# hir0shim/singleSpMV

Hardware: AMD Instinct MI355X
Metric: SpMV GFLOP/s (fp64) + achieved HBM GB/s (higher is better)
Workload: dtype f64

## Files before the change

### singlespmv_amd/csrc/k_bin.hip

```cpp
#include "device.hpp"
#include "internal.hpp"

namespace spmv {

typedef uint32_t bin_u32x4 __attribute__((ext_vector_type(4)));

template <int U>
struct MulBatch {
    double v[U];
    uint32_t c[U];
    int32_t d[U];
};

template <int U, int PL, int MODE, bool LONG>
__device__ __forceinline__ void mul_load(MulBatch<U> &B, int64_t base, int64_t e0, int64_t e1, int lane,
                                         const double *__restrict__ val1, const uint16_t *__restrict__ cs1,
                                         const int32_t *__restrict__ dst1, int64_t ls, int64_t lsh,
                                         const int32_t *__restrict__ lcode) {
    if constexpr (!LONG) {
        const double *vb = val1 + base + lane;
        const uint16_t *cb = cs1 + base + lane;
        const int32_t *db = dst1 + ((base + lane) >> PL);
#pragma unroll
        for (int u = 0; u < U; ++u) {
            B.v[u] = ld_stream(vb + u * 64);
            B.c[u] = (uint32_t)__builtin_nontemporal_load(cb + u * 64);
            if constexpr ((MODE & 4) == 0) B.d[u] = ld_stream(db + u * (64 >> PL));
        }
        (void)e0;
        (void)e1;
        (void)ls;
        (void)lsh;
        (void)lcode;
        (void)db;
    } else {
#pragma unroll
        for (int u = 0; u < U; ++u) {
            const int64_t e = base + u * 64 + lane;
            const int64_t ee = e < e1 ? e : e0;
            B.v[u] = ld_stream(val1 + ee);
            B.c[u] = (uint32_t)__builtin_nontemporal_load(cs1 + ee);
            if (base + u * 64 >= ls) B.d[u] = ld_stream(lcode + (e < e1 ? e + lsh : 0));
            else if constexpr ((MODE & 4) == 0) B.d[u] = ld_stream(dst1 + (ee >> PL));
        }
    }
}

__device__ __forceinline__ void mul_long_block(double pr, int32_t code, bool ok, int lane,
                                               double *__restrict__ prod) {
    const bool start = code < 0 || !ok;
    const uint64_t starts = __ballot(start);
    const uint64_t upto = starts & (~0ull >> (63 - lane));
    const int seg = 63 - __clzll((long long)upto);
    const int r16 = lane & 15, row = lane >> 4;
    double v = ok ? pr : 0.0, t;
    t = dpp_f64<0x111, 0xF>(v);
    if (r16 >= 1 && lane - 1 >= seg) v = __dadd_rn(t, v);
    t = dpp_f64<0x112, 0xF>(v);
    if (r16 >= 2 && lane - 2 >= seg) v = __dadd_rn(t, v);
    t = dpp_f64<0x114, 0xF>(v);
    if (r16 >= 4 && lane - 4 >= seg) v = __dadd_rn(t, v);
    t = dpp_f64<0x118, 0xF>(v);
    if (r16 >= 8 && lane - 8 >= seg) v = __dadd_rn(t, v);
    t = dpp_f64<0x142, 0xA>(v);
    if ((row & 1) && seg <= row * 16 - 1) v = __dadd_rn(t, v);
    t = dpp_f64<0x143, 0xC>(v);
    if (row >= 2 && seg <= 31) v = __dadd_rn(t, v);
    const int32_t pos = code & 0x7FFFFFFF;
    if (ok && pos != 0x7FFFFFFF) prod[pos] = v;
}

template <int U, int MODE, int PL, bool LONG>
__device__ __forceinline__ void mul_store(const MulBatch<U> &B, int64_t base, int64_t e1, int lane,
                                          const double *xs, double *__restrict__ prod, int64_t ls) {
#pragma unroll
    for (int u = 0; u < U; ++u) {
        const int64_t e = base + u * 64 + lane;
        if (LONG && base + u * 64 >= ls) {
            mul_long_block(__dmul_rn(B.v[u], xs[B.c[u]]), B.d[u], e < e1, lane, prod);
        } else if (e < e1) {
            const double pr = __dmul_rn(B.v[u], xs[B.c[u]]);
            double *dp = (MODE & 4) ? prod + e : prod + ((int64_t)B.d[u] << PL) + (e & ((1 << PL) - 1));
            if (MODE & 1) __builtin_nontemporal_store(pr, dp);
            else *dp = pr;
        }
    }
}

template <int U, int MODE, int PL, bool LONG>
__global__ __launch_bounds__(kBinMulThreads) void bin_mul_kernel(
    const int64_t *__restrict__ piece_off, int64_t q_base, const int32_t *__restrict__ piece_strip,
    const int64_t *__restrict__ piece_begin, const int64_t *__restrict__ piece_end,
    const double *__restrict__ val1, const uint16_t *__restrict__ cs1, const int32_t *__restrict__ dst1,
    const double *__restrict__ x, int64_t n, int32_t strip, double *__restrict__ prod,
    const int64_t *__restrict__ lstart, const int64_t *__restrict__ lshift, const int32_t *__restrict__ lcode,
    int32_t xburst) {
    __shared__ double xs[kBinMaxStrip];
    constexpr int NW = kBinMulThreads / 64;
    constexpr int64_t STEP = (int64_t)NW * 64 * U;
    const int w = __builtin_amdgcn_readfirstlane(threadIdx.x >> 6);
    const int lane = threadIdx.x & 63;
    const int64_t q0 = piece_off[q_base + blockIdx.x], q1 = piece_off[q_base + blockIdx.x + 1];
    for (int64_t q = q0; q < q1; ++q) {
        const int32_t st = piece_strip[q];
        const int64_t c0 = (int64_t)st * strip;
        const int64_t e0 = piece_begin[q], e1 = piece_end[q];
        const int64_t ls = LONG ? lstart[st] : INT64_MAX, lsh = LONG ? lshift[st] : 0;
        const int cw = (int)(n - c0 < strip ? n - c0 : strip);
        __syncthreads();
        constexpr int XL = 8;
        if constexpr ((MODE & 256) != 0) {
            const int full = cw & ~127;
            for (int k = w; k * 128 < full; k += NW)
                __builtin_amdgcn_global_load_lds(
                    (const __attribute__((address_space(1))) void *)(x + c0 + k * 128 + lane * 2),
                    (__attribute__((address_space(3))) void *)(xs + k * 128), 16, 0, 0);
            for (int i = full + threadIdx.x; i < cw; i += kBinMulThreads) xs[i] = x[c0 + i];
            __builtin_amdgcn_s_waitcnt(0x0F70);
        } else if (LONG || !xburst) {
            for (int i = threadIdx.x; i < cw; i += kBinMulThreads) xs[i] = x[c0 + i];
        } else for (int i0 = threadIdx.x; i0 < cw; i0 += XL * kBinMulThreads) {
            double t[XL];
#pragma unroll
            for (int k = 0; k < XL; ++k) {
                const int i = i0 + k * kBinMulThreads;
                t[k] = i < cw ? x[c0 + i] : 0.0;
            }
#pragma unroll
            for (int k = 0; k < XL; ++k) {
                const int i = i0 + k * kBinMulThreads;
                if (i < cw) xs[i] = t[k];
            }
        }
        __syncthreads();
        const int64_t first = e0 + (int64_t)w * 64 * U;
        const int64_t nit = first < e1 ? (e1 - first + STEP - 1) / STEP : 0;
        auto bat = [&](int64_t j) { return first + j * STEP; };
        MulBatch<U> A, B;
        if (nit > 0) mul_load<U, PL, MODE, LONG>(A, bat(0), e0, e1, lane, val1, cs1, dst1, ls, lsh, lcode);
        for (int64_t it = 0; it < nit; it += 2) {
            const int64_t ba = bat(it), bb = bat(it + 1);
            if (it + 1 < nit) mul_load<U, PL, MODE, LONG>(B, bb, e0, e1, lane, val1, cs1, dst1, ls, lsh, lcode);
            mul_store<U, MODE, PL, LONG>(A, ba, e1, lane, xs, prod, ls);
            if (it + 1 < nit) {
                if (it + 2 < nit)
                    mul_load<U, PL, MODE, LONG>(A, bat(it + 2), e0, e1, lane, val1, cs1, dst1, ls, lsh, lcode);
                mul_store<U, MODE, PL, LONG>(B, bb, e1, lane, xs, prod, ls);
            }
        }
    }
}

template <int U>
struct SumBatch {
    double v[U];
    uint32_t w[U / 2];
    __device__ __forceinline__ uint32_t slot(int u) const { return (w[u >> 1] >> (16 * (u & 1))) & 0xFFFFu; }
};

template <int U>
__device__ __forceinline__ void sum_load(SumBatch<U> &B, int64_t base, int lane, int64_t pbase, int64_t sbase,
                                         const uint16_t *__restrict__ slot2, const double *__restrict__ prod) {
    static_assert(U % 8 == 0, "slots are read 8 per 16-byte load");
    const bin_u32x4 *sp = reinterpret_cast<const bin_u32x4 *>(slot2 + sbase + (int64_t)lane * 8);
#pragma unroll
    for (int q = 0; q < U / 8; ++q) {
        const bin_u32x4 w = __builtin_nontemporal_load(sp + q * 64);
#pragma unroll
        for (int h = 0; h < 4; ++h) B.w[4 * q + h] = w[h];
    }
    const double *pp = prod + (base - pbase) + lane;
#pragma unroll
    for (int u = 0; u < U; ++u) B.v[u] = ld_stream(pp + u * 64);
}

template <int U>
__device__ __forceinline__ void sum_add(const SumBatch<U> &B, double *ys) {
#pragma unroll
    for (int u = 0; u < U; ++u) atomicAdd(&ys[B.slot(u)], B.v[u]);
}

template <int W2, int U>
__global__ __launch_bounds__(64 * W2) void bin_sum_kernel(
    int64_t b0, int64_t b1, int64_t nbins, int64_t nblk, const int64_t *__restrict__ run_off,
    const int64_t *__restrict__ srun_off, const int32_t *__restrict__ bin_row0, int64_t pbase,
    const uint16_t *__restrict__ slot2,
    const double *__restrict__ prod, double *__restrict__ y) {
    constexpr int SLICE = kBinLdsDoubles / W2;
    constexpr int64_t STEP = 64 * U;
    __shared__ double ylds[kBinLdsDoubles];
    const int w = __builtin_amdgcn_readfirstlane(threadIdx.x >> 6);
    const int lane = threadIdx.x & 63;
    double *ys = ylds + w * SLICE;
    const int64_t bfirst = b0 + (int64_t)blockIdx.x * W2 + w, bstride = (int64_t)gridDim.x * W2;
    if (bfirst >= b1) return;
    int64_t cb = bfirst, k = 0, pos = run_off[cb], end = run_off[cb + 1], rs = pos, ss = srun_off[cb];
    auto next = [&](int64_t &lo, int64_t &sb, int64_t &bb) -> bool {
        while (pos >= end) {
            if (++k >= nblk) {
                cb += bstride;
                if (cb >= b1) return false;
                k = 0;
                pos = rs = run_off[cb];
                end = run_off[cb + 1];
                ss = srun_off[cb];
                continue;
            }
            pos = rs = run_off[k * nbins + cb];
            end = run_off[k * nbins + cb + 1];
            ss = srun_off[k * nbins + cb];
        }
        lo = pos;
        sb = ss + (lo - rs);
        bb = cb;
        pos = pos + STEP < end ? pos + STEP : end;
        return true;
    };
    int64_t acc = -1, done = bfirst;
    auto write_zero = [&](int64_t bz) {
        const int64_t r0 = bin_row0[bz];
        const int rows = (int)(bin_row0[bz + 1] - r0);
        for (int i = lane; i < rows; i += 64) __builtin_nontemporal_store(0.0, y + r0 + i);
    };
    auto finish = [&]() {
        const int64_t r0 = bin_row0[acc];
        const int rows = (int)(bin_row0[acc + 1] - r0);
        __builtin_amdgcn_fence(__ATOMIC_SEQ_CST, "wavefront");
        for (int i = lane; i < rows; i += 64) __builtin_nontemporal_store(ys[i], y + r0 + i);
        __builtin_amdgcn_fence(__ATOMIC_SEQ_CST, "wavefront");
        done = acc + bstride;
    };
    auto begin = [&](int64_t nb) {
        if (nb == acc) return;
        if (acc >= 0) finish();
        for (; done < nb; done += bstride) write_zero(done);
        const int rows = (int)(bin_row0[nb + 1] - bin_row0[nb]);
        for (int i = lane; i < rows; i += 64) ys[i] = 0.0;
        acc = nb;
        done = nb + bstride;
    };
    SumBatch<U> A, B;
    int64_t alo, asb, ab, blo, bsb, bbn;
    bool has_a = next(alo, asb, ab);
    if (has_a) sum_load<U>(A, alo, lane, pbase, asb, slot2, prod);
    while (has_a) {
        const bool has_b = next(blo, bsb, bbn);
        if (has_b) sum_load<U>(B, blo, lane, pbase, bsb, slot2, prod);
        begin(ab);
        sum_add<U>(A, ys);
        if (!has_b) break;
        has_a = next(alo, asb, ab);
        if (has_a) sum_load<U>(A, alo, lane, pbase, asb, slot2, prod);
        begin(bbn);
        sum_add<U>(B, ys);
    }
    if (acc >= 0) finish();
    for (; done < b1; done += bstride) write_zero(done);
}

template <int U>
struct SumTab {
    int32_t t[U / 8];
};

template <int U>
__device__ __forceinline__ void sum_mo_tab(SumTab<U> &T, int64_t sb, int lane, const int32_t *__restrict__ mtab) {
    static_assert(U == 32, "U/8 = 4 table words per lane: one 16-byte load");
    const bin_u32x4 w = __builtin_nontemporal_load(reinterpret_cast<const bin_u32x4 *>(mtab + (sb >> 3)) + lane);
#pragma unroll
    for (int h = 0; h < 4; ++h) T.t[h] = (int32_t)w[h];
}

template <int U>
__device__ __forceinline__ void sum_mo_load(SumBatch<U> &B, const SumTab<U> &T, int64_t sb, int lane,
                                            const uint16_t *__restrict__ slot2, const double *__restrict__ prod) {
    const bin_u32x4 *sp = reinterpret_cast<const bin_u32x4 *>(slot2 + sb + (int64_t)lane * 8);
#pragma unroll
    for (int q = 0; q < U / 8; ++q) {
        const bin_u32x4 w = __builtin_nontemporal_load(sp + q * 64);
#pragma unroll
        for (int h = 0; h < 4; ++h) B.w[4 * q + h] = w[h];
    }
    const double *pl = prod + (lane & 7);
    int c[U];
#pragma unroll
    for (int u = 0; u < U; ++u) c[u] = __builtin_amdgcn_ds_bpermute((((u & 7) << 3) + (lane >> 3)) << 2, T.t[u >> 3]);
    __builtin_amdgcn_sched_barrier(0);
#pragma unroll
    for (int u = 0; u < U; ++u) B.v[u] = pl[c[u]];
}

template <int W2, int U>
__global__ __launch_bounds__(64 * W2) void bin_sum_bin_kernel(
    int64_t b0, int64_t b1, const int64_t *__restrict__ run_off, const int64_t *__restrict__ srun_off,
    const int32_t *__restrict__ bin_row0, const uint16_t *__restrict__ slot2, const int32_t *__restrict__ mtab,
    const double *__restrict__ prod, double *__restrict__ y) {
    constexpr int SLICE = kBinLdsDoubles / W2;
    constexpr int64_t STEP = 64 * U;
    __shared__ double ylds[kBinLdsDoubles];
    const int w = __builtin_amdgcn_readfirstlane(threadIdx.x >> 6);
    const int lane = threadIdx.x & 63;
    double *ys = ylds + w * SLICE;
    struct BinRun {
        int64_t r0 = 0, nb = 0, ss0 = 0;
        int rows = 0;
        __device__ int64_t s(int64_t j) const { return ss0 + j * STEP; }
    };
    auto bin_at = [&](int64_t b) {
        BinRun R;
        R.r0 = bin_row0[b];
        R.rows = (int)(bin_row0[b + 1] - R.r0);
        R.ss0 = srun_off[b];
        R.nb = (run_off[b + 1] - run_off[b] + STEP - 1) / STEP;
        return R;
    };
    const int64_t bstride = (int64_t)gridDim.x * W2;
    int64_t b = b0 + (int64_t)blockIdx.x * W2 + w;
    if (b >= b1) return;
    BinRun R = bin_at(b);
    for (int i = lane; i < R.rows; i += 64) ys[i] = 0.0;
    SumBatch<U> PA, PB;
    SumTab<U> TA, TB;
    bool pre = false;
    for (;;) {
        const int64_t bn = b + bstride;
        const bool more = bn < b1;
        const BinRun N = more ? bin_at(bn) : R;
        const bool pfn = more && N.nb > 0;
        auto sbat = [&](int64_t j) -> int64_t {
            if (j < R.nb) return R.s(j);
            return pfn ? N.s(j - R.nb < N.nb ? j - R.nb : N.nb - 1) : R.s(R.nb - 1);
        };
        bool swapped = false;
        if (R.nb > 0) {
            if (!pre) {
                sum_mo_tab<U>(TA, sbat(0), lane, mtab);
                sum_mo_tab<U>(TB, sbat(1), lane, mtab);
                sum_mo_load<U>(PA, TA, sbat(0), lane, slot2, prod);
            } else if (R.nb == 1) {
                sum_mo_tab<U>(TB, sbat(1), lane, mtab);
            }
            for (int64_t j = 0;; j += 2) {
                sum_mo_tab<U>(TA, sbat(j + 2), lane, mtab);
                sum_mo_load<U>(PB, TB, sbat(j + 1), lane, slot2, prod);
                sum_add<U>(PA, ys);
                if (j + 1 >= R.nb) {
                    swapped = true;
                    break;
                }
                sum_mo_tab<U>(TB, sbat(j + 3), lane, mtab);
                sum_mo_load<U>(PA, TA, sbat(j + 2), lane, slot2, prod);
                sum_add<U>(PB, ys);
                if (j + 2 >= R.nb) break;
            }
        }
        pre = R.nb > 0 && pfn;
        __builtin_amdgcn_fence(__ATOMIC_SEQ_CST, "wavefront");
        for (int i = lane; i < R.rows; i += 64) __builtin_nontemporal_store(ys[i], y + R.r0 + i);
        __builtin_amdgcn_fence(__ATOMIC_SEQ_CST, "wavefront");
        if (!more) break;
        for (int i = lane; i < N.rows; i += 64) ys[i] = 0.0;
        if (pre && swapped) {
            PA = PB;
            TB = TA;
        }
        b = bn;
        R = N;
    }
}

template <int W2>
static void launch_sum_mo(const spmv_plan_s *p, double *y) {
    const BinDev &B = p->bin;
    hipLaunchKernelGGL((bin_sum_bin_kernel<W2, 32>), dim3((unsigned)B.nwg2), dim3(64 * W2), 0, p->stream,
                       (int64_t)0, B.n_bins, B.run_off, B.srun_off, B.bin_row0, B.slot2, B.mtab, B.prod, y);
}

template <int MODE, int PL, int U = 8>
static void launch_mul_t(const spmv_plan_s *p, int g, const double *x) {
    const BinDev &B = p->bin;
    if (B.long_len > 0)
        hipLaunchKernelGGL((bin_mul_kernel<U, MODE, PL, true>), dim3((unsigned)B.nwg1), dim3(kBinMulThreads), 0,
                           p->stream, B.piece_off, (int64_t)g * B.nwg1, B.piece_strip, B.piece_begin, B.piece_end,
                           B.val1, B.cs1, B.dst1, x, p->n, (int32_t)B.strip, B.prod, B.lstart, B.lshift, B.lcode,
                           B.xburst);
    else
        hipLaunchKernelGGL((bin_mul_kernel<U, MODE, PL, false>), dim3((unsigned)B.nwg1), dim3(kBinMulThreads), 0,
                           p->stream, B.piece_off, (int64_t)g * B.nwg1, B.piece_strip, B.piece_begin, B.piece_end,
                           B.val1, B.cs1, B.dst1, x, p->n, (int32_t)B.strip, B.prod, nullptr, nullptr, nullptr,
                           B.xburst);
}

template <int PL>
static void launch_mul_p(const spmv_plan_s *p, int g, const double *x) {
    bool dma = (reinterpret_cast<uintptr_t>(x) & 15) == 0 && p->bin.strip % 2 == 0;
    if (launch_dbg(p->bin.dbg) & (1 << 24)) dma = false;
    if (p->bin.mo) {
        if (dma) launch_mul_t<256 | 4, PL>(p, g, x);
        else launch_mul_t<4, PL>(p, g, x);
    } else {
        if (dma) launch_mul_t<256 | 1, PL>(p, g, x);
        else launch_mul_t<1, PL>(p, g, x);
    }
}

static void launch_mul(const spmv_plan_s *p, int g, const double *x) {
    if (p->bin.pad_log == 5) launch_mul_p<5>(p, g, x);
    else if (p->bin.pad_log == 4) launch_mul_p<4>(p, g, x);
    else launch_mul_p<3>(p, g, x);
}

template <int W2, int U>
static void launch_sum_w(const spmv_plan_s *p, int g, double *y) {
    const BinDev &B = p->bin;
    const int64_t b0 = g < 0 ? 0 : B.g_bin[g], b1 = g < 0 ? B.n_bins : B.g_bin[g + 1];
    const int64_t pbase = g < 0 ? 0 : B.g_prod[g];
    hipLaunchKernelGGL((bin_sum_kernel<W2, U>), dim3((unsigned)B.nwg2), dim3(64 * W2), 0, p->stream, b0, b1,
                       B.n_bins, B.n_blocks, B.run_off, B.srun_off, B.bin_row0, pbase, B.slot2, B.prod, y);
}

int bin_time_mul(const spmv_plan_s *p, const double *x, float *ms) {
    const BinDev &B = p->bin;
    hipEvent_t a, b;
    SPMV_HIP_TRY(hipEventCreate(&a));
    SPMV_HIP_TRY(hipEventCreate(&b));
    for (int rep = 0; rep < 2; ++rep) {
        if (rep == 1) SPMV_HIP_TRY(hipEventRecord(a, p->stream));
        for (int g = 0; g < B.G; ++g) {
            launch_mul(p, g, x);
        }
    }
    SPMV_HIP_TRY(hipEventRecord(b, p->stream));
    SPMV_HIP_TRY(hipEventSynchronize(b));
    SPMV_HIP_TRY(hipEventElapsedTime(ms, a, b));
    (void)hipEventDestroy(a);
    (void)hipEventDestroy(b);
    return SPMV_SUCCESS;
}

int launch_bin(const spmv_plan_s *p, const double *x, double *y) {
    const BinDev &B = p->bin;
    if (p->m == 0) return SPMV_SUCCESS;
    if (p->nnz == 0) {
        SPMV_HIP_TRY(hipMemsetAsync(y, 0, sizeof(double) * (size_t)p->m, p->stream));
        return SPMV_SUCCESS;
    }
    auto sum = [&](int g) {
        if (B.mo) {
            if (B.sum_waves == 2) launch_sum_mo<2>(p, y);
            else launch_sum_mo<4>(p, y);
            return;
        }
        if (B.sum_waves == 2) launch_sum_w<2, 32>(p, g, y);
        else if (B.sum_waves == 4) launch_sum_w<4, 32>(p, g, y);
        else launch_sum_w<8, 8>(p, g, y);
    };
    for (int g = 0; g < B.G; ++g) {
        launch_mul(p, g, x);
        SPMV_HIP_TRY(hipGetLastError());
        if (B.reuse) {
            phase_mark(p);
            sum(g);
            SPMV_HIP_TRY(hipGetLastError());
            if (g + 1 < B.G) phase_mark(p);
        }
    }
    if (!B.reuse) {
        phase_mark(p);
        sum(-1);
        SPMV_HIP_TRY(hipGetLastError());
    }
    return SPMV_SUCCESS;
}

}
```

Before: 400.7.

## Vectorize bin handover: 16-byte LDS-to-HBM stores with fused zeroing and uniform table loads

Replaces the per-bin scalar copy of the LDS accumulator slice to y with a handover that aligns to 16 bytes, issues batched 2-double LDS reads and nontemporal global stores, and re-zeroes the LDS slots in the same pass. This drops the separate zeroing loop for the next bin and the wavefront fences. The bin walker is factored into a shared BinWalk struct, and table index loads are made wave-uniform through readfirstlane so they can become scalar loads. It adds head and tail handling complexity and assumes a 16-byte aligned LDS. The old kernels are kept behind a probe flag.

```diff
diff --git a/singlespmv_amd/csrc/bin_walk.hpp b/singlespmv_amd/csrc/bin_walk.hpp
--- /dev/null
+++ b/singlespmv_amd/csrc/bin_walk.hpp
@@ -0,0 +1,71 @@
+#pragma once
+#include <cstdint>
+
+#if defined(__HIPCC__) || defined(__CUDACC__)
+#define SPMV_WALK_HD __host__ __device__ __forceinline__
+#else
+#define SPMV_WALK_HD inline
+#endif
+
+namespace spmv {
+
+struct BinWalk {
+    int64_t b1 = 0, nbins = 0, nblk = 1, bstride = 1, step = 0;
+    int64_t cb = 0, k = 0, pos = 0, end = 0, rs = 0, ss = 0;
+    int64_t acc = -1, done = 0;
+
+    template <class Tab>
+    SPMV_WALK_HD void run_at(const Tab &t) {
+        const int64_t i = k * nbins + cb;
+        pos = rs = t.run(i);
+        end = t.run(i + 1);
+        ss = t.srun(i);
+    }
+
+    template <class Tab>
+    SPMV_WALK_HD bool start(const Tab &t, int64_t bfirst, int64_t b1_, int64_t nbins_, int64_t nblk_,
+                            int64_t bstride_, int64_t step_) {
+        b1 = b1_, nbins = nbins_, nblk = nblk_, bstride = bstride_, step = step_;
+        cb = done = bfirst;
+        acc = -1;
+        k = 0;
+        if (cb >= b1) return false;
+        run_at(t);
+        return true;
+    }
+
+    template <class Tab>
+    SPMV_WALK_HD bool next(const Tab &t, int64_t &lo, int64_t &sb, int64_t &bb) {
+        while (pos >= end) {
+            if (++k >= nblk) {
+                cb += bstride;
+                if (cb >= b1) return false;
+                k = 0;
+            }
+            run_at(t);
+        }
+        lo = pos;
+        sb = ss + (lo - rs);
+        bb = cb;
+        pos = pos + step < end ? pos + step : end;
+        return true;
+    }
+
+    template <class Handover, class Zeros>
+    SPMV_WALK_HD void begin(int64_t nb, Handover &&handover, Zeros &&zeros) {
+        if (nb == acc) return;
+        if (acc >= 0) handover(acc);
+        for (; done < nb; done += bstride) zeros(done);
+        acc = nb;
+        done = nb + bstride;
+    }
+
+    template <class Handover, class Zeros>
+    SPMV_WALK_HD void finish(Handover &&handover, Zeros &&zeros) {
+        if (acc >= 0) handover(acc);
+        acc = -1;
+        for (; done < b1; done += bstride) zeros(done);
+    }
+};
+
+}
diff --git a/singlespmv_amd/csrc/k_bin.hip b/singlespmv_amd/csrc/k_bin.hip
--- a/singlespmv_amd/csrc/k_bin.hip
+++ b/singlespmv_amd/csrc/k_bin.hip
@@ -1,5 +1,6 @@
 #include "device.hpp"
 #include "internal.hpp"
+#include "bin_walk.hpp"
 
 namespace spmv {
 
@@ -180,6 +181,73 @@
     for (int u = 0; u < U; ++u) atomicAdd(&ys[B.slot(u)], B.v[u]);
 }
 
+typedef double bin_f64x2 __attribute__((ext_vector_type(2)));
+typedef bin_f64x2 bin_f64x2_lds __attribute__((aligned(8)));
+
+template <int SLICE>
+__device__ __forceinline__ void sum_zero_slice(double *ys, int lane) {
+    static_assert(SLICE % 128 == 0, "whole 16-byte wave writes");
+    bin_f64x2 z = {0.0, 0.0};
+#pragma unroll
+    for (int s = 0; s < SLICE / 128; ++s) *reinterpret_cast<bin_f64x2 *>(ys + s * 128 + lane * 2) = z;
+}
+
+template <int SLICE>
+__device__ __forceinline__ void bin_handover(double *ys, int rows, double *__restrict__ y, int64_t r0, int lane) {
+    typedef __attribute__((address_space(1))) double gdouble;
+    typedef __attribute__((address_space(1))) bin_f64x2 gdouble2;
+    typedef __attribute__((address_space(3))) double ldouble;
+    typedef __attribute__((address_space(3))) bin_f64x2_lds ldouble2;
+    constexpr int NSTEP = (SLICE / 2 + 63) / 64, CH = 8;
+    const int head = (int)(((reinterpret_cast<uintptr_t>(y) >> 3) + (uint64_t)r0) & 1) & (rows > 0 ? 1 : 0);
+    const int nv = (rows - head) >> 1;
+    const bool tail = ((rows - head) & 1) != 0;
+    gdouble *yr = (gdouble *)y + r0;
+    {
+        const int i = lane == 0 ? 0 : lane == 1 ? rows - 1 : SLICE - 1;
+        const bool st = lane == 0 ? head != 0 : (lane == 1 && tail);
+        if (st || lane == 2) {
+            ldouble *yi = (ldouble *)ys + i;
+            const double v = *yi;
+            *yi = 0.0;
+            if (st) __builtin_nontemporal_store(v, yr + i);
+        }
+    }
+    ldouble *yl = (ldouble *)ys + head + lane * 2;
+    const bin_f64x2 z = {0.0, 0.0};
+#pragma unroll
+    for (int c = 0; c < NSTEP; c += CH) {
+        if (c * 64 >= nv) continue;
+        gdouble *yc = yr + head + c * 128;
+        bin_f64x2 v[CH];
+#pragma unroll
+        for (int s = 0; s < CH; ++s)
+            if (c + s < NSTEP)
+                v[s] = *(const ldouble2 *)((c + s) * 64 + lane < nv ? yl + (c + s) * 128 : yl + (c * 128 - lane * 2));
+#pragma unroll
+        for (int s = 0; s < CH; ++s)
+            if (c + s < NSTEP && (c + s) * 64 + lane < nv) {
+                *(ldouble2 *)(yl + (c + s) * 128) = z;
+                __builtin_nontemporal_store(v[s], (gdouble2 *)(yc + (uint32_t)(lane * 2 + s * 128)));
+            }
+    }
+}
+
+__device__ __forceinline__ int64_t sum_uni(int64_t v) {
+    const uint32_t lo = (uint32_t)__builtin_amdgcn_readfirstlane((int)(uint32_t)v);
+    const uint32_t hi = (uint32_t)__builtin_amdgcn_readfirstlane((int)(uint32_t)((uint64_t)v >> 32));
+    return (int64_t)(((uint64_t)hi << 32) | lo);
+}
+
+struct SumTabs {
+    const int64_t *__restrict__ run_off;
+    const int64_t *__restrict__ srun_off;
+    const int32_t *__restrict__ bin_row0;
+    __device__ __forceinline__ int64_t run(int64_t i) const { return run_off[sum_uni(i)]; }
+    __device__ __forceinline__ int64_t srun(int64_t i) const { return srun_off[sum_uni(i)]; }
+    __device__ __forceinline__ int64_t row0(int64_t b) const { return (int64_t)bin_row0[sum_uni(b)]; }
+};
+
 template <int W2, int U>
 __global__ __launch_bounds__(64 * W2) void bin_sum_kernel(
     int64_t b0, int64_t b1, int64_t nbins, int64_t nblk, const int64_t *__restrict__ run_off,
@@ -188,74 +256,41 @@
     const double *__restrict__ prod, double *__restrict__ y) {
     constexpr int SLICE = kBinLdsDoubles / W2;
     constexpr int64_t STEP = 64 * U;
-    __shared__ double ylds[kBinLdsDoubles];
+    __shared__ __attribute__((aligned(16))) double ylds[kBinLdsDoubles];
     const int w = __builtin_amdgcn_readfirstlane(threadIdx.x >> 6);
     const int lane = threadIdx.x & 63;
     double *ys = ylds + w * SLICE;
-    const int64_t bfirst = b0 + (int64_t)blockIdx.x * W2 + w, bstride = (int64_t)gridDim.x * W2;
-    if (bfirst >= b1) return;
-    int64_t cb = bfirst, k = 0, pos = run_off[cb], end = run_off[cb + 1], rs = pos, ss = srun_off[cb];
-    auto next = [&](int64_t &lo, int64_t &sb, int64_t &bb) -> bool {
-        while (pos >= end) {
-            if (++k >= nblk) {
-                cb += bstride;
-                if (cb >= b1) return false;
-                k = 0;
-                pos = rs = run_off[cb];
-                end = run_off[cb + 1];
-                ss = srun_off[cb];
-                continue;
-            }
-            pos = rs = run_off[k * nbins + cb];
-            end = run_off[k * nbins + cb + 1];
-            ss = srun_off[k * nbins + cb];
-        }
-        lo = pos;
-        sb = ss + (lo - rs);
-        bb = cb;
-        pos = pos + STEP < end ? pos + STEP : end;
-        return true;
-    };
-    int64_t acc = -1, done = bfirst;
-    auto write_zero = [&](int64_t bz) {
-        const int64_t r0 = bin_row0[bz];
-        const int rows = (int)(bin_row0[bz + 1] - r0);
+    const SumTabs T{run_off, srun_off, bin_row0};
+    BinWalk W;
+    if (!W.start(T, b0 + (int64_t)blockIdx.x * W2 + w, b1, nbins, nblk, (int64_t)gridDim.x * W2, STEP)) return;
+    auto zeros = [&](int64_t bz) __attribute__((always_inline)) {
+        const int64_t r0 = T.row0(bz);
+        const int rows = (int)(T.row0(bz + 1) - r0);
         for (int i = lane; i < rows; i += 64) __builtin_nontemporal_store(0.0, y + r0 + i);
     };
-    auto finish = [&]() {
-        const int64_t r0 = bin_row0[acc];
-        const int rows = (int)(bin_row0[acc + 1] - r0);
-        __builtin_amdgcn_fence(__ATOMIC_SEQ_CST, "wavefront");
-        for (int i = lane; i < rows; i += 64) __builtin_nontemporal_store(ys[i], y + r0 + i);
-        __builtin_amdgcn_fence(__ATOMIC_SEQ_CST, "wavefront");
-        done = acc + bstride;
+    auto handover = [&](int64_t bf) __attribute__((always_inline)) {
+        const int64_t r0 = T.row0(bf);
+        const int rows = (int)(T.row0(bf + 1) - r0);
+        bin_handover<SLICE>(ys, rows, y, r0, lane);
     };
-    auto begin = [&](int64_t nb) {
-        if (nb == acc) return;
-        if (acc >= 0) finish();
-        for (; done < nb; done += bstride) write_zero(done);
-        const int rows = (int)(bin_row0[nb + 1] - bin_row0[nb]);
-        for (int i = lane; i < rows; i += 64) ys[i] = 0.0;
-        acc = nb;
-        done = nb + bstride;
-    };
+    auto begin = [&](int64_t nb) __attribute__((always_inline)) { W.begin(nb, handover, zeros); };
     SumBatch<U> A, B;
     int64_t alo, asb, ab, blo, bsb, bbn;
-    bool has_a = next(alo, asb, ab);
+    bool has_a = W.next(T, alo, asb, ab);
     if (has_a) sum_load<U>(A, alo, lane, pbase, asb, slot2, prod);
+    sum_zero_slice<SLICE>(ys, lane);
     while (has_a) {
-        const bool has_b = next(blo, bsb, bbn);
+        const bool has_b = W.next(T, blo, bsb, bbn);
         if (has_b) sum_load<U>(B, blo, lane, pbase, bsb, slot2, prod);
         begin(ab);
         sum_add<U>(A, ys);
         if (!has_b) break;
-        has_a = next(alo, asb, ab);
+        has_a = W.next(T, alo, asb, ab);
         if (has_a) sum_load<U>(A, alo, lane, pbase, asb, slot2, prod);
         begin(bbn);
         sum_add<U>(B, ys);
     }
-    if (acc >= 0) finish();
-    for (; done < b1; done += bstride) write_zero(done);
+    W.finish(handover, zeros);
 }
 
 template <int U>
@@ -297,7 +332,7 @@
     const double *__restrict__ prod, double *__restrict__ y) {
     constexpr int SLICE = kBinLdsDoubles / W2;
     constexpr int64_t STEP = 64 * U;
-    __shared__ double ylds[kBinLdsDoubles];
+    __shared__ __attribute__((aligned(16))) double ylds[kBinLdsDoubles];
     const int w = __builtin_amdgcn_readfirstlane(threadIdx.x >> 6);
     const int lane = threadIdx.x & 63;
     double *ys = ylds + w * SLICE;
@@ -306,19 +341,20 @@
         int rows = 0;
         __device__ int64_t s(int64_t j) const { return ss0 + j * STEP; }
     };
+    const SumTabs T{run_off, srun_off, bin_row0};
     auto bin_at = [&](int64_t b) {
         BinRun R;
-        R.r0 = bin_row0[b];
-        R.rows = (int)(bin_row0[b + 1] - R.r0);
-        R.ss0 = srun_off[b];
-        R.nb = (run_off[b + 1] - run_off[b] + STEP - 1) / STEP;
+        R.r0 = T.row0(b);
+        R.rows = (int)(T.row0(b + 1) - R.r0);
+        R.ss0 = T.srun(b);
+        R.nb = (T.run(b + 1) - T.run(b) + STEP - 1) / STEP;
         return R;
     };
     const int64_t bstride = (int64_t)gridDim.x * W2;
     int64_t b = b0 + (int64_t)blockIdx.x * W2 + w;
     if (b >= b1) return;
     BinRun R = bin_at(b);
-    for (int i = lane; i < R.rows; i += 64) ys[i] = 0.0;
+    sum_zero_slice<SLICE>(ys, lane);
     SumBatch<U> PA, PB;
     SumTab<U> TA, TB;
     bool pre = false;
@@ -355,11 +391,8 @@
             }
         }
         pre = R.nb > 0 && pfn;
-        __builtin_amdgcn_fence(__ATOMIC_SEQ_CST, "wavefront");
-        for (int i = lane; i < R.rows; i += 64) __builtin_nontemporal_store(ys[i], y + R.r0 + i);
-        __builtin_amdgcn_fence(__ATOMIC_SEQ_CST, "wavefront");
+        bin_handover<SLICE>(ys, R.rows, y, R.r0, lane);
         if (!more) break;
-        for (int i = lane; i < N.rows; i += 64) ys[i] = 0.0;
         if (pre && swapped) {
             PA = PB;
             TB = TA;
@@ -369,9 +402,20 @@
     }
 }
 
+#ifdef SPMV_PROBES
+#include "k_bin_prev.inc"
+#endif
+
 template <int W2>
 static void launch_sum_mo(const spmv_plan_s *p, double *y) {
     const BinDev &B = p->bin;
+#ifdef SPMV_PROBES
+    if (launch_dbg(B.dbg) & (1 << 25)) {
+        hipLaunchKernelGGL((bin_sum_bin_kernel_prev<W2, 32>), dim3((unsigned)B.nwg2), dim3(64 * W2), 0, p->stream,
+                           (int64_t)0, B.n_bins, B.run_off, B.srun_off, B.bin_row0, B.slot2, B.mtab, B.prod, y);
+        return;
+    }
+#endif
     hipLaunchKernelGGL((bin_sum_bin_kernel<W2, 32>), dim3((unsigned)B.nwg2), dim3(64 * W2), 0, p->stream,
                        (int64_t)0, B.n_bins, B.run_off, B.srun_off, B.bin_row0, B.slot2, B.mtab, B.prod, y);
 }
@@ -415,6 +459,13 @@
     const BinDev &B = p->bin;
     const int64_t b0 = g < 0 ? 0 : B.g_bin[g], b1 = g < 0 ? B.n_bins : B.g_bin[g + 1];
     const int64_t pbase = g < 0 ? 0 : B.g_prod[g];
+#ifdef SPMV_PROBES
+    if (launch_dbg(B.dbg) & (1 << 25)) {
+        hipLaunchKernelGGL((bin_sum_kernel_prev<W2, U>), dim3((unsigned)B.nwg2), dim3(64 * W2), 0, p->stream, b0, b1,
+                           B.n_bins, B.n_blocks, B.run_off, B.srun_off, B.bin_row0, pbase, B.slot2, B.prod, y);
+        return;
+    }
+#endif
     hipLaunchKernelGGL((bin_sum_kernel<W2, U>), dim3((unsigned)B.nwg2), dim3(64 * W2), 0, p->stream, b0, b1,
                        B.n_bins, B.n_blocks, B.run_off, B.srun_off, B.bin_row0, pbase, B.slot2, B.prod, y);
 }
diff --git a/singlespmv_amd/csrc/k_bin_prev.inc b/singlespmv_amd/csrc/k_bin_prev.inc
--- /dev/null
+++ b/singlespmv_amd/csrc/k_bin_prev.inc
@@ -0,0 +1,157 @@
+
+template <int W2, int U>
+__global__ __launch_bounds__(64 * W2) void bin_sum_kernel_prev(
+    int64_t b0, int64_t b1, int64_t nbins, int64_t nblk, const int64_t *__restrict__ run_off,
+    const int64_t *__restrict__ srun_off, const int32_t *__restrict__ bin_row0, int64_t pbase,
+    const uint16_t *__restrict__ slot2,
+    const double *__restrict__ prod, double *__restrict__ y) {
+    constexpr int SLICE = kBinLdsDoubles / W2;
+    constexpr int64_t STEP = 64 * U;
+    __shared__ double ylds[kBinLdsDoubles];
+    const int w = __builtin_amdgcn_readfirstlane(threadIdx.x >> 6);
+    const int lane = threadIdx.x & 63;
+    double *ys = ylds + w * SLICE;
+    const int64_t bfirst = b0 + (int64_t)blockIdx.x * W2 + w, bstride = (int64_t)gridDim.x * W2;
+    if (bfirst >= b1) return;
+    int64_t cb = bfirst, k = 0, pos = run_off[cb], end = run_off[cb + 1], rs = pos, ss = srun_off[cb];
+    auto next = [&](int64_t &lo, int64_t &sb, int64_t &bb) -> bool {
+        while (pos >= end) {
+            if (++k >= nblk) {
+                cb += bstride;
+                if (cb >= b1) return false;
+                k = 0;
+                pos = rs = run_off[cb];
+                end = run_off[cb + 1];
+                ss = srun_off[cb];
+                continue;
+            }
+            pos = rs = run_off[k * nbins + cb];
+            end = run_off[k * nbins + cb + 1];
+            ss = srun_off[k * nbins + cb];
+        }
+        lo = pos;
+        sb = ss + (lo - rs);
+        bb = cb;
+        pos = pos + STEP < end ? pos + STEP : end;
+        return true;
+    };
+    int64_t acc = -1, done = bfirst;
+    auto write_zero = [&](int64_t bz) {
+        const int64_t r0 = bin_row0[bz];
+        const int rows = (int)(bin_row0[bz + 1] - r0);
+        for (int i = lane; i < rows; i += 64) __builtin_nontemporal_store(0.0, y + r0 + i);
+    };
+    auto finish = [&]() {
+        const int64_t r0 = bin_row0[acc];
+        const int rows = (int)(bin_row0[acc + 1] - r0);
+        __builtin_amdgcn_fence(__ATOMIC_SEQ_CST, "wavefront");
+        for (int i = lane; i < rows; i += 64) __builtin_nontemporal_store(ys[i], y + r0 + i);
+        __builtin_amdgcn_fence(__ATOMIC_SEQ_CST, "wavefront");
+        done = acc + bstride;
+    };
+    auto begin = [&](int64_t nb) {
+        if (nb == acc) return;
+        if (acc >= 0) finish();
+        for (; done < nb; done += bstride) write_zero(done);
+        const int rows = (int)(bin_row0[nb + 1] - bin_row0[nb]);
+        for (int i = lane; i < rows; i += 64) ys[i] = 0.0;
+        acc = nb;
+        done = nb + bstride;
+    };
+    SumBatch<U> A, B;
+    int64_t alo, asb, ab, blo, bsb, bbn;
+    bool has_a = next(alo, asb, ab);
+    if (has_a) sum_load<U>(A, alo, lane, pbase, asb, slot2, prod);
+    while (has_a) {
+        const bool has_b = next(blo, bsb, bbn);
+        if (has_b) sum_load<U>(B, blo, lane, pbase, bsb, slot2, prod);
+        begin(ab);
+        sum_add<U>(A, ys);
+        if (!has_b) break;
+        has_a = next(alo, asb, ab);
+        if (has_a) sum_load<U>(A, alo, lane, pbase, asb, slot2, prod);
+        begin(bbn);
+        sum_add<U>(B, ys);
+    }
+    if (acc >= 0) finish();
+    for (; done < b1; done += bstride) write_zero(done);
+}
+
+template <int W2, int U>
+__global__ __launch_bounds__(64 * W2) void bin_sum_bin_kernel_prev(
+    int64_t b0, int64_t b1, const int64_t *__restrict__ run_off, const int64_t *__restrict__ srun_off,
+    const int32_t *__restrict__ bin_row0, const uint16_t *__restrict__ slot2, const int32_t *__restrict__ mtab,
+    const double *__restrict__ prod, double *__restrict__ y) {
+    constexpr int SLICE = kBinLdsDoubles / W2;
+    constexpr int64_t STEP = 64 * U;
+    __shared__ double ylds[kBinLdsDoubles];
+    const int w = __builtin_amdgcn_readfirstlane(threadIdx.x >> 6);
+    const int lane = threadIdx.x & 63;
+    double *ys = ylds + w * SLICE;
+    struct BinRun {
+        int64_t r0 = 0, nb = 0, ss0 = 0;
+        int rows = 0;
+        __device__ int64_t s(int64_t j) const { return ss0 + j * STEP; }
+    };
+    auto bin_at = [&](int64_t b) {
+        BinRun R;
+        R.r0 = bin_row0[b];
+        R.rows = (int)(bin_row0[b + 1] - R.r0);
+        R.ss0 = srun_off[b];
+        R.nb = (run_off[b + 1] - run_off[b] + STEP - 1) / STEP;
+        return R;
+    };
+    const int64_t bstride = (int64_t)gridDim.x * W2;
+    int64_t b = b0 + (int64_t)blockIdx.x * W2 + w;
+    if (b >= b1) return;
+    BinRun R = bin_at(b);
+    for (int i = lane; i < R.rows; i += 64) ys[i] = 0.0;
+    SumBatch<U> PA, PB;
+    SumTab<U> TA, TB;
+    bool pre = false;
+    for (;;) {
+        const int64_t bn = b + bstride;
+        const bool more = bn < b1;
+        const BinRun N = more ? bin_at(bn) : R;
+        const bool pfn = more && N.nb > 0;
+        auto sbat = [&](int64_t j) -> int64_t {
+            if (j < R.nb) return R.s(j);
+            return pfn ? N.s(j - R.nb < N.nb ? j - R.nb : N.nb - 1) : R.s(R.nb - 1);
+        };
+        bool swapped = false;
+        if (R.nb > 0) {
+            if (!pre) {
+                sum_mo_tab<U>(TA, sbat(0), lane, mtab);
+                sum_mo_tab<U>(TB, sbat(1), lane, mtab);
+                sum_mo_load<U>(PA, TA, sbat(0), lane, slot2, prod);
+            } else if (R.nb == 1) {
+                sum_mo_tab<U>(TB, sbat(1), lane, mtab);
+            }
+            for (int64_t j = 0;; j += 2) {
+                sum_mo_tab<U>(TA, sbat(j + 2), lane, mtab);
+                sum_mo_load<U>(PB, TB, sbat(j + 1), lane, slot2, prod);
+                sum_add<U>(PA, ys);
+                if (j + 1 >= R.nb) {
+                    swapped = true;
+                    break;
+                }
+                sum_mo_tab<U>(TB, sbat(j + 3), lane, mtab);
+                sum_mo_load<U>(PA, TA, sbat(j + 2), lane, slot2, prod);
+                sum_add<U>(PB, ys);
+                if (j + 2 >= R.nb) break;
+            }
+        }
+        pre = R.nb > 0 && pfn;
+        __builtin_amdgcn_fence(__ATOMIC_SEQ_CST, "wavefront");
+        for (int i = lane; i < R.rows; i += 64) __builtin_nontemporal_store(ys[i], y + R.r0 + i);
+        __builtin_amdgcn_fence(__ATOMIC_SEQ_CST, "wavefront");
+        if (!more) break;
+        for (int i = lane; i < N.rows; i += 64) ys[i] = 0.0;
+        if (pre && swapped) {
+            PA = PB;
+            TB = TA;
+        }
+        b = bn;
+        R = N;
+    }
+}
```

New measurement: 402.0 (median of 6 runs). Within noise of the previous version (+0.3%).

## Restructure bin sum kernel loads with scalar bases, constant-space tables, vector writeback

Applied to the files above, without the earlier changes.

Rewrites the bin-sum kernel's streaming loads to use wave-uniform scalar base pointers plus per-lane VGPR offsets, with scheduling barriers to keep the loads issued in order. It reads run and row offset tables through the constant address space and precomputes batch counts, which simplifies the next-batch logic. LDS zeroing and writeback to y now use 16-byte vector accesses, and the wavefront fences around the writeback are removed. The intent is to cut address arithmetic, VGPR pressure and instruction count in a memory-bound phase. The risks are correctness of the batch-count logic when runs are empty or partial, and the sched barriers limiting how the compiler interleaves work.

```diff
diff --git a/singlespmv_amd/csrc/k_bin.hip b/singlespmv_amd/csrc/k_bin.hip
--- a/singlespmv_amd/csrc/k_bin.hip
+++ b/singlespmv_amd/csrc/k_bin.hip
@@ -159,25 +159,81 @@
 };
 
 template <int U>
-__device__ __forceinline__ void sum_load(SumBatch<U> &B, int64_t base, int lane, int64_t pbase, int64_t sbase,
+struct SumStream {
+    double v[U];
+    bin_u32x4 w[U / 8];
+    uint32_t so, po;
+    __device__ __forceinline__ uint32_t slot(int u) const {
+        return (w[u >> 3][(u >> 1) & 3] >> (16 * (u & 1))) & 0xFFFFu;
+    }
+};
+
+typedef const __attribute__((address_space(1))) char *bin_gptr;
+__device__ __forceinline__ bin_gptr sgpr_ptr(const void *p) {
+    const uint64_t a = reinterpret_cast<uint64_t>(p);
+    const uint32_t lo = __builtin_amdgcn_readfirstlane((uint32_t)a);
+    const uint32_t hi = __builtin_amdgcn_readfirstlane((uint32_t)(a >> 32));
+    return (bin_gptr)(((uint64_t)hi << 32) | lo);
+}
+
+template <int U>
+__device__ __forceinline__ void sum_load(SumStream<U> &B, int64_t base, int lane, int64_t pbase, int64_t sbase,
                                          const uint16_t *__restrict__ slot2, const double *__restrict__ prod) {
     static_assert(U % 8 == 0, "slots are read 8 per 16-byte load");
-    const bin_u32x4 *sp = reinterpret_cast<const bin_u32x4 *>(slot2 + sbase + (int64_t)lane * 8);
+    const bin_gptr sp = sgpr_ptr(slot2 + sbase), pp = sgpr_ptr(prod + (base - pbase));
+    typedef const __attribute__((address_space(1))) bin_u32x4 *gslots;
+    typedef const __attribute__((address_space(1))) double *gprods;
+    uint32_t &so = B.so, &po = B.po;
+    asm volatile("" : "+v"(so), "+v"(po));
+    __builtin_amdgcn_sched_barrier(0);
 #pragma unroll
     for (int q = 0; q < U / 8; ++q) {
-        const bin_u32x4 w = __builtin_nontemporal_load(sp + q * 64);
-#pragma unroll
-        for (int h = 0; h < 4; ++h) B.w[4 * q + h] = w[h];
-    }
-    const double *pp = prod + (base - pbase) + lane;
-#pragma unroll
-    for (int u = 0; u < U; ++u) B.v[u] = ld_stream(pp + u * 64);
-}
-
-template <int U>
-__device__ __forceinline__ void sum_add(const SumBatch<U> &B, double *ys) {
+        B.w[q] = __builtin_nontemporal_load((gslots)(sp + (size_t)so + q * 1024));
+        __builtin_amdgcn_sched_barrier(0);
+    }
+#pragma unroll
+    for (int u = 0; u < U; ++u) {
+        B.v[u] = __builtin_nontemporal_load((gprods)(pp + (size_t)po + u * 512));
+        __builtin_amdgcn_sched_barrier(0);
+    }
+}
+
+template <int U, class Batch>
+__device__ __forceinline__ void sum_add(const Batch &B, double *ys) {
 #pragma unroll
     for (int u = 0; u < U; ++u) atomicAdd(&ys[B.slot(u)], B.v[u]);
+}
+
+__device__ __forceinline__ void sum_write_back(const double *ys, double *__restrict__ yp, int rows, int lane) {
+    if ((reinterpret_cast<uintptr_t>(yp) & 15) == 0) {
+        for (int i0 = 2 * lane; i0 < rows; i0 += 512) {
+            f64x2 t[4];
+#pragma unroll
+            for (int j = 0; j < 4; ++j) t[j] = *reinterpret_cast<const f64x2 *>(ys + i0 + 128 * j);
+#pragma unroll
+            for (int j = 0; j < 4; ++j) {
+                const int i = i0 + 128 * j;
+                if (i + 1 < rows) __builtin_nontemporal_store(t[j], reinterpret_cast<f64x2 *>(yp + i));
+                else if (i < rows) __builtin_nontemporal_store(t[j].x, yp + i);
+            }
+        }
+    } else {
+        for (int i0 = lane; i0 < rows; i0 += 512) {
+            double t[8];
+#pragma unroll
+            for (int j = 0; j < 8; ++j) t[j] = ys[i0 + 64 * j];
+#pragma unroll
+            for (int j = 0; j < 8; ++j)
+                if (i0 + 64 * j < rows) __builtin_nontemporal_store(t[j], yp + i0 + 64 * j);
+        }
+    }
+}
+
+__device__ __forceinline__ void sum_zero_slice(double *ys, int rows, int lane) {
+    f64x2 z;
+    z.x = 0.0;
+    z.y = 0.0;
+    for (int i = 2 * lane; i < rows; i += 128) *reinterpret_cast<f64x2 *>(ys + i) = z;
 }
 
 template <int W2, int U>
@@ -188,73 +244,84 @@
     const double *__restrict__ prod, double *__restrict__ y) {
     constexpr int SLICE = kBinLdsDoubles / W2;
     constexpr int64_t STEP = 64 * U;
-    __shared__ double ylds[kBinLdsDoubles];
+    static_assert(SLICE % 512 == 0, "sum_write_back reads whole 512-row trips inside the slice");
+    __shared__ __attribute__((aligned(16))) double ylds[kBinLdsDoubles];
     const int w = __builtin_amdgcn_readfirstlane(threadIdx.x >> 6);
     const int lane = threadIdx.x & 63;
     double *ys = ylds + w * SLICE;
     const int64_t bfirst = b0 + (int64_t)blockIdx.x * W2 + w, bstride = (int64_t)gridDim.x * W2;
     if (bfirst >= b1) return;
-    int64_t cb = bfirst, k = 0, pos = run_off[cb], end = run_off[cb + 1], rs = pos, ss = srun_off[cb];
+    typedef const __attribute__((address_space(4))) int64_t *ctab64;
+    typedef const __attribute__((address_space(4))) int32_t *ctab32;
+    const ctab64 run = (ctab64)run_off, srun = (ctab64)srun_off;
+    const ctab32 row0 = (ctab32)bin_row0;
+    auto batches = [&](int64_t i) { return (int64_t)((uint64_t)(run[i + 1] - run[i] + STEP - 1) / (uint64_t)STEP); };
+    int64_t cb = bfirst, k = 0, pos = run[cb], ss = srun[cb], left = batches(cb);
+    int64_t bins = (b1 - bfirst + bstride - 1) / bstride;
     auto next = [&](int64_t &lo, int64_t &sb, int64_t &bb) -> bool {
-        while (pos >= end) {
-            if (++k >= nblk) {
+        while (left == 0) {
+            if (++k == nblk) {
+                if (--bins == 0) return false;
                 cb += bstride;
-                if (cb >= b1) return false;
                 k = 0;
-                pos = rs = run_off[cb];
-                end = run_off[cb + 1];
-                ss = srun_off[cb];
-                continue;
-            }
-            pos = rs = run_off[k * nbins + cb];
-            end = run_off[k * nbins + cb + 1];
-            ss = srun_off[k * nbins + cb];
+            }
+            pos = run[k * nbins + cb];
+            ss = srun[k * nbins + cb];
+            left = batches(k * nbins + cb);
         }
         lo = pos;
-        sb = ss + (lo - rs);
+        sb = ss;
         bb = cb;
-        pos = pos + STEP < end ? pos + STEP : end;
+        pos += STEP;
+        ss += STEP;
+        --left;
         return true;
     };
     int64_t acc = -1, done = bfirst;
     auto write_zero = [&](int64_t bz) {
-        const int64_t r0 = bin_row0[bz];
-        const int rows = (int)(bin_row0[bz + 1] - r0);
+        const int64_t r0 = row0[bz];
+        const int rows = (int)(row0[bz + 1] - r0);
         for (int i = lane; i < rows; i += 64) __builtin_nontemporal_store(0.0, y + r0 + i);
     };
     auto finish = [&]() {
-        const int64_t r0 = bin_row0[acc];
-        const int rows = (int)(bin_row0[acc + 1] - r0);
-        __builtin_amdgcn_fence(__ATOMIC_SEQ_CST, "wavefront");
-        for (int i = lane; i < rows; i += 64) __builtin_nontemporal_store(ys[i], y + r0 + i);
-        __builtin_amdgcn_fence(__ATOMIC_SEQ_CST, "wavefront");
+        const int64_t r0 = row0[acc];
+        sum_write_back(ys, y + r0, (int)(row0[acc + 1] - r0), lane);
         done = acc + bstride;
     };
     auto begin = [&](int64_t nb) {
         if (nb == acc) return;
         if (acc >= 0) finish();
         for (; done < nb; done += bstride) write_zero(done);
-        const int rows = (int)(bin_row0[nb + 1] - bin_row0[nb]);
-        for (int i = lane; i < rows; i += 64) ys[i] = 0.0;
+        sum_zero_slice(ys, (int)(row0[nb + 1] - row0[nb]), lane);
         acc = nb;
         done = nb + bstride;
     };
-    SumBatch<U> A, B;
+    SumStream<U> A, B;
+    A.so = B.so = (uint32_t)lane * 16u;
+    A.po = B.po = (uint32_t)lane * 8u;
     int64_t alo, asb, ab, blo, bsb, bbn;
-    bool has_a = next(alo, asb, ab);
-    if (has_a) sum_load<U>(A, alo, lane, pbase, asb, slot2, prod);
-    while (has_a) {
-        const bool has_b = next(blo, bsb, bbn);
-        if (has_b) sum_load<U>(B, blo, lane, pbase, bsb, slot2, prod);
-        begin(ab);
-        sum_add<U>(A, ys);
-        if (!has_b) break;
-        has_a = next(alo, asb, ab);
-        if (has_a) sum_load<U>(A, alo, lane, pbase, asb, slot2, prod);
-        begin(bbn);
-        sum_add<U>(B, ys);
-    }
-    if (acc >= 0) finish();
+    if (next(alo, asb, ab)) {
+        sum_load<U>(A, alo, lane, pbase, asb, slot2, prod);
+        for (;;) {
+            if (!next(blo, bsb, bbn)) {
+                begin(ab);
+                sum_add<U>(A, ys);
+                break;
+            }
+            sum_load<U>(B, blo, lane, pbase, bsb, slot2, prod);
+            begin(ab);
+            sum_add<U>(A, ys);
+            if (!next(alo, asb, ab)) {
+                begin(bbn);
+                sum_add<U>(B, ys);
+                break;
+            }
+            sum_load<U>(A, alo, lane, pbase, asb, slot2, prod);
+            begin(bbn);
+            sum_add<U>(B, ys);
+        }
+        finish();
+    }
     for (; done < b1; done += bstride) write_zero(done);
 }
 
```

New measurement: 392.2 before, 383.9 after. -2.1%, worse.
